# RKWin93/E2E-MAPPO-for-MT-FJSP

Hardware: AMD Instinct MI355X
Metric: env-steps/sec (batched J6M6E2) (higher is better)
Workload: dtype f64 (environment) / f32 (encoder: f32 storage and accumulation; 128x128 products on the 16-bit matrix cores from split f32 operands, f32-accurate: DESIGN.md §4)

## Files before the change

### __graft_entry__.py

```python
#!/usr/bin/env python3
import os
import sys

ROOT = os.path.dirname(os.path.abspath(__file__))
if ROOT not in sys.path:
    sys.path.insert(0, ROOT)


def build() -> None:
    from importlib import import_module
    import mtfjsp_amd
    _build = import_module("e2e-mappo-for-mt-fjsp_amd._build")
    lib = _build.build(force=True, verbose=True)
    capi = import_module("e2e-mappo-for-mt-fjsp_amd.capi")
    capi.lib()
    print("variant:", _build.build_variant("funcs", ["-DMTFJSP_BODY_FUNCS=3"]))
    from oracle import env_oracle
    print("oracle:", env_oracle.build(force=True))
    print("built", lib)


def smoke() -> None:
    import numpy as np
    import torch
    from importlib import import_module
    import mtfjsp_amd
    assert torch.cuda.is_available(), "smoke() needs cuda:0"
    batch_env = import_module("e2e-mappo-for-mt-fjsp_amd.batch_env")
    inst = import_module("e2e-mappo-for-mt-fjsp_amd.instances")
    from oracle.env_oracle import OracleBatch
    J, M, E, B = 6, 6, 2, 8
    T = J * M
    t, p, tt, edge = inst.generate_instances(B, J, M, E, seed=0)
    import random
    random.seed(0)
    w3 = inst.random_weights(B)
    env = batch_env.DeviceBatchEnv(J, M, E, B, obs_dtype="f64")
    env.load_instances(t, p, tt, edge=edge)
    env.scaler_init()
    env.reset(w3)
    orc = OracleBatch(t, p, tt, edge)
    orc.scaler_init()
    orc.reset(w3)
    a = torch.zeros(B, dtype=torch.int32, device=env.device); m = torch.zeros_like(a); j = torch.zeros_like(a)
    for s in range(T):
        env.random_actions(7, s, a, m, j)
        env.step(a, m)
        info, raw, _ = orc.step(a.cpu().numpy(), m.cpu().numpy())
        cand, mask = orc.job_mask_update(j.cpu().numpy())
# ... 25 lines not shown
```

### e2e-mappo-for-mt-fjsp_amd/csrc/mtfjsp_gin_resident.h

```cpp
#ifndef GR_KERNEL
#ifndef MTFJSP_GIN_RESIDENT_H
#define MTFJSP_GIN_RESIDENT_H
#include <type_traits>
#include <utility>
#include "mtfjsp_gin_res_select.h"

#ifndef GR_ABL
#define GR_ABL 0
#endif
#ifndef GR_NRES
#define GR_NRES 16
#endif
#ifndef GR_VRES
#define GR_VRES 1
#endif
#define GR_RING 6
#define GR_NBAR 6
#ifndef GR_GRP
#define GR_GRP 2
#endif
#ifndef GR_LOOK
#define GR_LOOK 2
#endif
#define GR_ROWB 272
#define GR_PLANE (32 * GR_ROWB)
#define GR_TILE (2 * GR_PLANE)
#define GR_MAXWARM 10
#ifndef GR_FX_DROP
#define GR_FX_DROP 1
#endif
#ifndef GR_FX_TAIL
#define GR_FX_TAIL 1
#endif
#ifndef GR_FX_SETUP
#define GR_FX_SETUP 1
#endif
struct GrShapeAny { static constexpr bool FIXED = false; static constexpr int T = 0, J = 0, IPC = 0; };
template <int T_, int J_, int IPC_> struct GrShapeFixed {
    static constexpr bool FIXED = true; static constexpr int T = T_, J = J_, IPC = IPC_;
    static_assert(T_ >= GR_MINT && T_ <= GR_MAXT && IPC_ * T_ == GR_ROWS && IPC_ * J_ <= GR_MAXCAND && (IPC_ * 128) % 256 == 0, "fixed shape: full 576-row workgroups");
};
typedef GrShapeFixed<GIN_RES_FX_T, GIN_RES_FX_J, GIN_RES_FX_IPC> GrShapeHeadline;
constexpr int gr_left_at(int T, int h, int rt)
{
    int left = ((16 * h) / T + 1) * T - 16 * h;
    for (int i = 0; i < rt; i++) { left -= 32; if (left <= 0) left += T; if (left <= 0) left += T; }
    return left;
}
constexpr int gr_max_chunks(int T)
{
    int m = 0;
    for (int i = 0; i < 16; i++) { const int r0 = i * T, c = ((r0 + T - 1) >> 4) - (r0 >> 4) + 1; m = c > m ? c : m; }
    return m;
}

#ifndef GR_MIX
#define GR_MIX 2
#endif
#ifndef GR_SETTLE
#define GR_SETTLE 1
#endif
#ifndef GR_FOLD_DPP
#define GR_FOLD_DPP 1
#endif
#ifndef GR_STAT_ASM
#define GR_STAT_ASM 0
#endif
#ifndef GR_PK
#define GR_PK 1
#endif
typedef float f32x16 __attribute__((ext_vector_type(16)));
typedef _Float16 gr_h8 __attribute__((ext_vector_type(8)));
typedef _Float16 gr_h2 __attribute__((ext_vector_type(2)));

struct GinResArgs {
    int B, T, J, ipc;
    const void *tfea; int feat_f64;
    const int *ell_col; const float *ell_val;
    const void *Wx32[6];
    float wsinv[6];
    const float *gamma[6], *beta[6];
    unsigned long long *stats;
    unsigned long long *stats_next;
    int wexp[6];
    int ffrac[6];
    unsigned long long *bar;
    unsigned long long epoch;
    unsigned *fail;
    unsigned *range_flag;
    const int *candidate;
    float *pooled;
    float *cand_feat;
    float *h_nodes;
// ... 218 lines not shown
            if (r < GR_ROWS) {
                unsigned cp = 0xffffffffu; float v0 = 0.f, v1 = 0.f;
                if (r < nrows) {
                    const int2 cc = ecc[k];
                    const float2 vv = evv[k];
                    const int base = (r / T) * T;
                    const unsigned r0 = cc.x >= 0 ? (unsigned)(base + cc.x) : 0xffffu, r1 = cc.y >= 0 ? (unsigned)(base + cc.y) : 0xffffu;
                    cp = r0 | (r1 << 16); v0 = cc.x >= 0 ? vv.x : 0.f; v1 = cc.y >= 0 ? vv.y : 0.f;
                }
                s_ellc[r] = cp; s_ellv0[r] = v0; s_ellv1[r] = v1; s_rowcand[r] = -1;
            }
        }
        {
            const f32x4 *wi = reinterpret_cast<const f32x4 *>(A.Wx32[0]) + (size_t)wave * (3 * 64) + lane;
            __builtin_amdgcn_sched_barrier(0);
#pragma unroll
            for (int p = 0; p < 3; p++) w0pre[p] = wi[p * 64];
            __builtin_amdgcn_sched_barrier(0);
        }
        if (tid == 0) s_flag[1] = 0u;
        if (tid < 5 * (GR_NT / GR_GRP)) s_cnt[tid] = 0u;
        for (int i = tid; i < 2 * GR_TILE / 16; i += 256) reinterpret_cast<float4 *>(s_planes)[i] = make_float4(0.f, 0.f, 0.f, 0.f);
        if (have_cand) {
            LDS_BARRIER();
#pragma unroll
            for (int k = 0; k < (GR_MAXCAND + 255) / 256; k++) {
                const int i = tid + 256 * k, c = cand_pre[k];
                if (i < ninst * Jn && c >= 0 && c < T && atomicExch(&s_rowcand[(i / Jn) * T + c], i) != -1) s_flag[1] = 1u;
            }
        }
        if constexpr (!FXD) s_zero[tid] = 0.f;
    }
    f32x16 acc[GR_NRES];
    f32x16 zs[2];
    float *zsp = A.zspill + ((size_t)(blockIdx.x * 4 + wave) * (GR_NT - GR_NRES)) * 1024 + lane * 4;
    auto zload = [&](auto Jc) __attribute__((always_inline)) {
        constexpr int j = decltype(Jc)::value;
        if constexpr (GR_VRES) return;
#pragma unroll
        for (int g = 0; g < 4; g++) {
            const float4 v = *reinterpret_cast<const float4 *>(zsp + j * 1024 + g * 256);
            zs[j & 1][4 * g] = v.x; zs[j & 1][4 * g + 1] = v.y; zs[j & 1][4 * g + 2] = v.z; zs[j & 1][4 * g + 3] = v.w;
        }
    };
    auto zstore = [&](auto Jc, const f32x16 &a) __attribute__((always_inline)) {
        constexpr int j = decltype(Jc)::value;
        if constexpr (GR_VRES) return;
#pragma unroll
        for (int g = 0; g < 4; g++) *reinterpret_cast<float4 *>(zsp + j * 1024 + g * 256) = make_float4(a[4 * g], a[4 * g + 1], a[4 * g + 2], a[4 * g + 3]);
    };
#define GR_TILEVAL(rt) ((rt) < GR_NRES ? acc[(rt) < GR_NRES ? (rt) : 0] : zs[(rt) >= GR_NRES ? ((rt) - GR_NRES) & 1 : 0])
    auto mfma_v = [&](f32x16 &c, const gr_h8 &a, const gr_h8 &b, bool zero) __attribute__((always_inline)) {
        if (zero) asm volatile("v_mfma_f32_32x32x16_f16 %0, %1, %2, 0" : "=v"(c) : "v"(a), "v"(b));
        else asm volatile("v_mfma_f32_32x32x16_f16 %0, %1, %2, %0" : "+v"(c) : "v"(a), "v"(b));
    };
    int nrows_l = nrows, n_l = n;
    auto bn_of = [&](int rt) __attribute__((always_inline)) -> const float * {
        if constexpr (FXD) return s_bn;
        else return rt * 32 + n_l < nrows_l ? s_bn : s_zero;
    };
    bool timed_out = false;
    gr_h8 wf[2][8];
    bf16x8 w0f[3];
    f32x2 ts[8], tq[8];
#pragma unroll
    for (int i = 0; i < 8; i++) { ts[i] = f32x2{0.f, 0.f}; tq[i] = f32x2{0.f, 0.f}; }

    auto load_weights = [&](int layer) __attribute__((always_inline)) {
        const float4 *wi = reinterpret_cast<const float4 *>(A.Wx32[layer]) + (size_t)wave * (2 * 8 * 64) + lane;
#pragma unroll
        for (int p = 0; p < 2; p++)
#pragma unroll
            for (int ks = 0; ks < 8; ks++) wf[p][ks] = __builtin_bit_cast(gr_h8, wi[(p * 8 + ks) * 64]);
    };
    auto stat2 = [&](int i, float x, float y) __attribute__((always_inline)) {
        const f32x2 v = {x, y};
#if GR_STAT_ASM == 1
        asm volatile("v_pk_add_f32 %0, %2, %0\n\tv_pk_fma_f32 %1, %2, %2, %1" : "+v"(ts[i]), "+v"(tq[i]) : "v"(v));
#elif GR_STAT_ASM == 2
        float s0 = ts[i][0], s1 = ts[i][1], q0 = tq[i][0], q1 = tq[i][1];
        asm volatile("v_add_f32 %0, %4, %0\n\tv_add_f32 %1, %5, %1\n\tv_fma_f32 %2, %4, %4, %2\n\tv_fma_f32 %3, %5, %5, %3" : "+v"(s0), "+v"(s1), "+v"(q0), "+v"(q1) : "v"(x), "v"(y));
        ts[i] = f32x2{s0, s1}; tq[i] = f32x2{q0, q1};
#else
        ts[i] = gr_add2(ts[i], v); tq[i] = gr_fma2(v, v, tq[i]);
        asm volatile("" : "+v"(ts[i]), "+v"(tq[i]));
#endif
    };
    auto stats_all = [&](const f32x16 &a) __attribute__((always_inline)) {
        if (GR_ABL & 4) return;
#pragma unroll
        for (int i = 0; i < 8; i++) stat2(i, a[2 * i], a[2 * i + 1]);
    };
    auto split2x4 = [&](f32x2 v01, f32x2 v23, uint2 &p0, uint2 &p1) __attribute__((always_inline)) {
        const gr_h2 a = __builtin_convertvector(v01, gr_h2), b = __builtin_convertvector(v23, gr_h2);
#if GR_MIX == 2
        const gr_h2 c = gr_rem16(v01, a), d = gr_rem16(v23, b);
#else
        const f32x2 r01 = gr_rem2(v01, a), r23 = gr_rem2(v23, b);
        const gr_h2 c = __builtin_convertvector(r01, gr_h2), d = __builtin_convertvector(r23, gr_h2);
#endif
        p0 = make_uint2(__builtin_bit_cast(unsigned, a), __builtin_bit_cast(unsigned, b));
        p1 = make_uint2(__builtin_bit_cast(unsigned, c), __builtin_bit_cast(unsigned, d));
    };
    auto stats_tile = [&](auto Tc) __attribute__((always_inline)) {
        constexpr int RT = decltype(Tc)::value;
        stats_all(GR_TILEVAL(RT));
// ... 18 lines not shown
    };
    auto fold_stats_dpp = [&]() __attribute__((always_inline)) {
        const bool b4 = (lane & 16) != 0, b3 = (lane & 8) != 0, b2 = (lane & 4) != 0, b1 = (lane & 2) != 0, b0 = (lane & 1) != 0;
        auto dpp = [&](float x, auto Ctrl) __attribute__((always_inline)) {
            return __builtin_bit_cast(float, __builtin_amdgcn_update_dpp(0, __builtin_bit_cast(int, x), decltype(Ctrl)::value, 0xF, 0xF, true));
        };
        float v16[16];
#pragma unroll
        for (int c = 0; c < 16; c++) {
            const float a = ts[c >> 1][c & 1], q_ = tq[c >> 1][c & 1];
            v16[c] = (b4 ? q_ : a) + __shfl_xor(b4 ? a : q_, 16);
        }
#pragma unroll
        for (int i = 0; i < 8; i++) { ts[i] = f32x2{0.f, 0.f}; tq[i] = f32x2{0.f, 0.f}; }
        float v8[8];
#pragma unroll
        for (int c = 0; c < 8; c++) v8[c] = (b3 ? v16[c + 8] : v16[c]) + dpp(b3 ? v16[c] : v16[c + 8], std::integral_constant<int, 0x140>{});
        float v4[4];
#pragma unroll
        for (int c = 0; c < 4; c++) v4[c] = (b2 ? v8[c + 4] : v8[c]) + dpp(b2 ? v8[c] : v8[c + 4], std::integral_constant<int, 0x141>{});
        float v2[2];
#pragma unroll
        for (int c = 0; c < 2; c++) v2[c] = (b1 ? v4[c + 2] : v4[c]) + dpp(b1 ? v4[c] : v4[c + 2], std::integral_constant<int, 0x4E>{});
        return (b0 ? v2[1] : v2[0]) + dpp(b0 ? v2[0] : v2[1], std::integral_constant<int, 0xB1>{});
    };
    unsigned char *const pl0 = s_planes, *const pl1 = s_planes + GR_TILE, *const plr = reinterpret_cast<unsigned char *>(s_ring);
    auto plane_buf = [&](int i) __attribute__((always_inline)) { return i == 0 ? pl0 : i == 1 ? pl1 : plr + (i - 2) * GR_TILE; };
    auto produce_quarter = [&](auto Tc, auto Gc, unsigned char *pbuf) __attribute__((always_inline)) {
        constexpr int rt = decltype(Tc)::value, g = decltype(Gc)::value;
        unsigned char *dst = pbuf + n * GR_ROWB + (32 * wave + 8 * g + 4 * h) * 2;
        const float *bn = bn_of(rt);
        const float4 s4 = *reinterpret_cast<const float4 *>(bn + 32 * wave + 8 * g + 4 * h);
        const float4 h4 = *reinterpret_cast<const float4 *>(bn + HD + 32 * wave + 8 * g + 4 * h);
        const f32x16 &a = GR_TILEVAL(rt);
        uint2 p0, p1;
        split2x4(f32x2{bn_relu_ss(a[4 * g], s4.x, h4.x), bn_relu_ss(a[4 * g + 1], s4.y, h4.y)},
                 f32x2{bn_relu_ss(a[4 * g + 2], s4.z, h4.z), bn_relu_ss(a[4 * g + 3], s4.w, h4.w)}, p0, p1);
        *reinterpret_cast<uint2 *>(dst) = p0;
        *reinterpret_cast<uint2 *>(dst + GR_PLANE) = p1;
    };
    auto produce_tile = [&](auto Tc, unsigned char *pbuf) __attribute__((always_inline)) {
        gr_static_for<4>([&](auto Gc) __attribute__((always_inline)) { produce_quarter(Tc, Gc, pbuf); });
        __builtin_amdgcn_sched_barrier(0);
    };
    const unsigned char *xa0 = s_planes + n * GR_ROWB + 16 * h;
#define GR_FENCE() __builtin_amdgcn_sched_barrier(0)
#define GR_PIN_V() do { } while (0)
    auto consume_tile = [&](auto Tc) __attribute__((always_inline)) {
        constexpr int RT = decltype(Tc)::value;
        constexpr int PT = RT + GR_LOOK;
        constexpr bool NEXT = (PT < GR_NT) && !(GR_ABL & 1);
        constexpr bool STATS = RT > 0 && (GR_VRES || RT - 1 < GR_NRES) && !(GR_ABL & 4);
        const unsigned char *xa = plane_buf(RT % (2 * GR_LOOK)) + n * GR_ROWB + 16 * h;
        unsigned char *pnext = plane_buf(PT % (2 * GR_LOOK));
        const float *bn = bn_of(PT);
        gr_h8 xf[2][2];
#pragma unroll
        for (int p = 0; p < 2; p++) xf[0][p] = *reinterpret_cast<const gr_h8 *>(xa + p * GR_PLANE);
        float4 s4 = make_float4(0.f, 0.f, 0.f, 0.f), h4 = s4;
        if constexpr (NEXT) {
            s4 = *reinterpret_cast<const float4 *>(bn + 32 * wave + 4 * h);
            h4 = *reinterpret_cast<const float4 *>(bn + HD + 32 * wave + 4 * h);
        }
        constexpr bool VT = GR_VRES && RT >= GR_NRES;
        f32x16 atmp;
        f32x16 &a = RT < GR_NRES ? acc[RT < GR_NRES ? RT : 0] : VT ? zs[RT >= GR_NRES ? (RT - GR_NRES) & 1 : 0] : atmp;
        if constexpr (RT + GR_LOOK + 1 >= GR_NRES && RT + GR_LOOK + 1 < GR_NT) zload(std::integral_constant<int, RT + GR_LOOK + 1 - GR_NRES>{});
        gr_static_for<4>([&](auto Pc) __attribute__((always_inline)) {
            constexpr int g = decltype(Pc)::value;
            const gr_h8 *x0 = xf[0], *x1 = xf[1];
            f32x2 v01 = {0.f, 0.f}, v23 = {0.f, 0.f}, e01 = v01, e23 = v01;
            gr_h2 p01 = {0, 0}, p23 = p01, q01 = p01, q23 = p01;
            unsigned char *dst = pnext + n * GR_ROWB + (32 * wave + 8 * g + 4 * h) * 2;
            const f32x16 &nx = GR_TILEVAL(PT < GR_NT ? PT : RT);
            const f32x16 &pv = GR_TILEVAL(RT > 0 ? RT - 1 : 0);
            auto M = [&](int ks, int wp, int xp) __attribute__((always_inline)) {
                if (GR_ABL & 2) return;
                if constexpr (VT) mfma_v(a, wf[wp][ks], (ks & 1) ? x1[xp] : x0[xp], ks == 0 && wp == 0 && xp == 1);
                else if (ks == 0 && wp == 0 && xp == 1)
                    a = __builtin_amdgcn_mfma_f32_32x32x16_f16(wf[wp][ks], x0[xp], f32x16{0.f, 0.f, 0.f, 0.f, 0.f, 0.f, 0.f, 0.f, 0.f, 0.f, 0.f, 0.f, 0.f, 0.f, 0.f, 0.f}, 0, 0, 0);
                else a = __builtin_amdgcn_mfma_f32_32x32x16_f16(wf[wp][ks], (ks & 1) ? x1[xp] : x0[xp], a, 0, 0, 0);
            };
            M(2 * g, 0, 1);
            xf[1][0] = *reinterpret_cast<const gr_h8 *>(xa + 32 * (2 * g + 1));
            if constexpr (NEXT) { v01 = gr_fma2(f32x2{nx[4 * g], nx[4 * g + 1]}, f32x2{s4.x, s4.y}, f32x2{h4.x, h4.y});
                                  v23 = gr_fma2(f32x2{nx[4 * g + 2], nx[4 * g + 3]}, f32x2{s4.z, s4.w}, f32x2{h4.z, h4.w}); }
            GR_FENCE();
            M(2 * g, 1, 0);
            xf[1][1] = *reinterpret_cast<const gr_h8 *>(xa + GR_PLANE + 32 * (2 * g + 1));
            if constexpr (NEXT) { v01 = __builtin_elementwise_max(v01, f32x2{0.f, 0.f}); v23 = __builtin_elementwise_max(v23, f32x2{0.f, 0.f}); }
            GR_FENCE();
            M(2 * g, 0, 0);
            if constexpr (NEXT) { p01 = __builtin_convertvector(v01, gr_h2); p23 = __builtin_convertvector(v23, gr_h2); }
            if constexpr (NEXT && g < 3) s4 = *reinterpret_cast<const float4 *>(bn + 32 * wave + 8 * (g + 1) + 4 * h);
            GR_FENCE();
            M(2 * g + 1, 0, 1);
            if constexpr (g < 3) xf[0][0] = *reinterpret_cast<const gr_h8 *>(xa + 32 * (2 * g + 2));
            if constexpr (NEXT && !GR_MIX) { e01 = __builtin_convertvector(p01, f32x2); e23 = __builtin_convertvector(p23, f32x2); }
            if constexpr (NEXT && g < 3) h4 = *reinterpret_cast<const float4 *>(bn + HD + 32 * wave + 8 * (g + 1) + 4 * h);
            GR_FENCE();
            M(2 * g + 1, 1, 0);
            if constexpr (g < 3) xf[0][1] = *reinterpret_cast<const gr_h8 *>(xa + GR_PLANE + 32 * (2 * g + 2));
            if constexpr (NEXT) { if constexpr (GR_MIX == 2) { q01 = gr_rem16(v01, p01); q23 = gr_rem16(v23, p23); }
                                  else if constexpr (GR_MIX == 1) { v01 = gr_rem2(v01, p01); v23 = gr_rem2(v23, p23); } else { v01 = gr_sub2(v01, e01); v23 = gr_sub2(v23, e23); }
                                  if (!(GR_ABL & 8)) *reinterpret_cast<uint2 *>(dst) = make_uint2(__builtin_bit_cast(unsigned, p01), __builtin_bit_cast(unsigned, p23));
                                  if constexpr (GR_MIX != 2) { q01 = __builtin_convertvector(v01, gr_h2); q23 = __builtin_convertvector(v23, gr_h2); } }
            GR_FENCE();
            M(2 * g + 1, 0, 0);
            if constexpr (NEXT) { if (!(GR_ABL & 8)) *reinterpret_cast<uint2 *>(dst + GR_PLANE) = make_uint2(__builtin_bit_cast(unsigned, q01), __builtin_bit_cast(unsigned, q23));
                                  else asm volatile("" :: "v"(p01), "v"(p23), "v"(q01), "v"(q23)); }
            if constexpr (STATS) { stat2(2 * g, pv[4 * g], pv[4 * g + 1]); stat2(2 * g + 1, pv[4 * g + 2], pv[4 * g + 3]); }
            GR_FENCE();
        });
        if constexpr (RT >= GR_NRES && !GR_VRES) {
            stats_all(a);
            zstore(std::integral_constant<int, RT - GR_NRES>{}, a);
            GR_FENCE();
        }
        if constexpr (!VT && GR_SETTLE) { asm volatile("s_nop 1"); GR_FENCE(); }
    };
    auto consume_tile0 = [&](auto Tc) __attribute__((always_inline)) {
        constexpr int RT = decltype(Tc)::value;
        const unsigned char *xa = xa0 + 32 * (RT & 7);
        bf16x8 x[3];
#pragma unroll
        for (int p = 0; p < 3; p++) x[p] = *reinterpret_cast<const bf16x8 *>(xa + p * GR_PLANE);
        f32x16 a = {0.f, 0.f, 0.f, 0.f, 0.f, 0.f, 0.f, 0.f, 0.f, 0.f, 0.f, 0.f, 0.f, 0.f, 0.f, 0.f};
        a = __builtin_amdgcn_mfma_f32_32x32x16_bf16(w0f[0], x[2], a, 0, 0, 0);
        a = __builtin_amdgcn_mfma_f32_32x32x16_bf16(w0f[2], x[0], a, 0, 0, 0);
        a = __builtin_amdgcn_mfma_f32_32x32x16_bf16(w0f[1], x[1], a, 0, 0, 0);
        a = __builtin_amdgcn_mfma_f32_32x32x16_bf16(w0f[0], x[1], a, 0, 0, 0);
        a = __builtin_amdgcn_mfma_f32_32x32x16_bf16(w0f[1], x[0], a, 0, 0, 0);
        a = __builtin_amdgcn_mfma_f32_32x32x16_bf16(w0f[0], x[0], a, 0, 0, 0);
        if constexpr (RT < GR_NRES) acc[RT] = a;
        else if constexpr (GR_VRES) zs[(RT - GR_NRES) & 1] = a;
        else {
            stats_all(a);
            zstore(std::integral_constant<int, RT - GR_NRES>{}, a);
        }
        if constexpr (RT > 0 && (GR_VRES || RT - 1 < GR_NRES)) stats_tile(std::integral_constant<int, RT - 1>{});
        __builtin_amdgcn_sched_barrier(0);
    };
    float *s_wtab = s_ring + 1024 + 4 * (2 * 32 * 36);
    static_assert(!(GR_FX_SETUP && GR_FOLD_DPP) || (1024 + 4 * (2 * 32 * 36)) * 4 >= (2 * GR_LOOK - 2) * GR_TILE, "s_wtab lies past the plane buffers in the ring area");
    unsigned warm_word = 0;
    int slot[GR_NT];
    auto final_setup_a = [&]() __attribute__((always_inline)) {
        int tid_s = tid;
        if constexpr (FXS) asm volatile("" : "+v"(tid_s));
        for (int i = tid_s; i < 17 * 16; i += 256) s_wtab[i] = (i & 15) < (i >> 4) ? 1.0f : 0.0f;
        if (A.nwarm > 0) {
            unsigned l = (blockIdx.x >> 3) * 256u + (unsigned)tid_s;
            const unsigned char *wp = reinterpret_cast<const unsigned char *>(A.warm[0]);
            bool found = false;
            for (int w = 0; w < A.nwarm; w++) {
                const unsigned nl = A.warm_lines[w];
                if (!found && l < nl) { wp = reinterpret_cast<const unsigned char *>(A.warm[w]) + (size_t)l * 128; found = true; }
                if (!found) l -= nl;
            }
            warm_word = *reinterpret_cast<const unsigned *>(wp);
        }
    };
    auto final_setup_b = [&]() __attribute__((always_inline)) {
#ifndef GR_KEEP_MASKS
        asm volatile("" : "+v"(n_l));
#endif
#pragma unroll
        for (int rt = 0; rt < GR_NT; rt++) slot[rt] = (GR_ABL & 32) ? -1 : s_rowcand[rt * 32 + n_l];
    };
    auto layer_boundary = [&](auto Kc) __attribute__((always_inline)) {
        constexpr int k = decltype(Kc)::value;
        GR_STAMP_AT(4 + 4 * k);
        if constexpr (GR_VRES && GR_NT > GR_NRES) {
            asm volatile("s_nop 15\n\ts_nop 15" ::: "memory");
            stats_all(zs[(GR_NT - 1 - GR_NRES) & 1]);
        }
#if GR_FOLD_DPP
        (void)fold_stats;
        const float colsum = fold_stats_dpp();
        int lane_b = lane;
        if constexpr (FXS && k == 5) asm volatile("" : "+v"(lane_b));
        const int n_b = lane_b & 31, h_b = lane_b >> 5;
        const int kind = n_b >> 4, scol = 32 * wave + 8 * ((n_b & 15) >> 2) + 4 * h_b + (n_b & 3);
        constexpr int PAIR = 16;
#else
        const float colsum = fold_stats();
        const int kind = tid & 1, scol = tid >> 1;
        constexpr int PAIR = 1;
#endif
        const int sidx = 2 * scol + kind;
        if (k == 1) GR_STAMP_AT(2);
        const unsigned grp = blockIdx.x & 7u;
        {
            float x = colsum;
            if (!(__builtin_fabsf(x) * (kind ? A.wsinv[k] * A.wsinv[k] : A.wsinv[k]) < __builtin_ldexpf(1.0f, 51 - A.ffrac[k]))) {
                if (A.range_flag && !timed_out) __hip_atomic_store(A.range_flag, 1u, __ATOMIC_RELAXED, __HIP_MEMORY_SCOPE_SYSTEM);
                x = 0.f;
            }
            (void)__hip_atomic_fetch_add(A.stats + ((size_t)k * 8 + grp) * 256 + sidx, gr_fix_encode(x, kind ? 2 * A.wexp[k] : A.wexp[k], A.ffrac[k]),
                                         __ATOMIC_RELAXED, __HIP_MEMORY_SCOPE_AGENT);
        }
        if (k == 1) GR_STAMP_AT(3);
        const float ga = A.gamma[k][scol], be = A.beta[k][scol];
        if constexpr (k < 5) load_weights(k + 1);
        else if constexpr (FXS) { final_setup_a(); final_setup_b(); }
        GR_STAMP_AT(5 + 4 * k);
        const unsigned long long *w0 = A.stats + (size_t)k * 8 * 256 + sidx;
        unsigned long long vw[8], want[8], ssum = 0;
#pragma unroll
        for (int j = 0; j < 8; j++) want[j] = (unsigned long long)((nblk >> 3) + ((unsigned)j < (nblk & 7u) ? 1u : 0u));
        {
            const unsigned long long t0 = __builtin_amdgcn_s_memrealtime();
            for (;;) {
#pragma unroll
                for (int j = 0; j < 8; j++) vw[j] = __hip_atomic_load(w0 + (size_t)j * 256, __ATOMIC_RELAXED, __HIP_MEMORY_SCOPE_AGENT);
                bool done = true;
                ssum = 0;
#pragma unroll
                for (int j = 0; j < 8; j++) { done = done && (vw[j] >> 58) == want[j]; ssum += vw[j] & GR_FIX_PAYLOAD; }
                if (__builtin_amdgcn_ballot_w64(!done) == 0ull) break;
                if (__builtin_amdgcn_s_memrealtime() - t0 > 400000ull) {
                    __hip_atomic_store(A.fail, 1u, __ATOMIC_RELAXED, __HIP_MEMORY_SCOPE_SYSTEM);
                    timed_out = true;
                    break;
                }
                __builtin_amdgcn_s_sleep(2);
            }
            GR_STAMP_AT(6 + 4 * k);
            const double tot = gr_fix_decode(ssum, nblk, A.ffrac[k]);
            const double oth = __shfl_xor(tot, PAIR);
            if (!kind) {
                const double mean = tot * A.inv_rows;
                double var = oth * A.inv_rows - mean * mean;
                if (var < 0) var = 0;
                const float rstd = 1.0f / sqrtf((float)(var + BN_EPS));
                const float s = rstd * ga;
                s_bn[scol] = s * A.wsinv[k];
                s_bn[HD + scol] = be - (float)mean * s;
            }
        }
        LDS_BARRIER();
        GR_STAMP_AT(7 + 4 * k);
    };

    GR_STAMP_AT(0);
#pragma unroll
    for (int p = 0; p < 3; p++) w0f[p] = __builtin_bit_cast(bf16x8, w0pre[p]);
    LDS_BARRIER();
    GR_STAMP_AT(1);
    {
        const float *s_feat = s_ring;
        auto produce0 = [&](int rt) __attribute__((always_inline)) {
            const int r = 8 * wave + (lane >> 3), fk = lane & 7, row = rt * 32 + r;
            const int fo = fk < 6 ? 2 * fk : 0;
            const unsigned cp = s_ellc[row];
            const unsigned r0 = cp & 0xffffu, r1 = cp >> 16;
            const int deg = 1 + (r0 != 0xffffu) + (r1 != 0xffffu);
            const float inv = deg == 1 ? 1.0f : deg == 2 ? 0.5f : (1.0f / 3.0f);
            const float w0 = s_ellv0[row], w1 = s_ellv1[row];
            const int n0 = r0 != 0xffffu ? (int)r0 : row, n1 = r1 != 0xffffu ? (int)r1 : row;
            const float2 o = *reinterpret_cast<const float2 *>(s_feat + row * 12 + fo);
            const float2 x = *reinterpret_cast<const float2 *>(s_feat + n0 * 12 + fo);
            const float2 y = *reinterpret_cast<const float2 *>(s_feat + n1 * 12 + fo);
            float v[4] = {__builtin_fmaf(w1, y.x, __builtin_fmaf(w0, x.x, o.x)) * inv, __builtin_fmaf(w1, y.y, __builtin_fmaf(w0, x.y, o.y)) * inv, 0.f, 0.f};
            if (!FXD && row >= nrows) { v[0] = 0.f; v[1] = 0.f; }
            uint2 p0, p1, p2;
            split3x4(v, p0, p1, p2);
            unsigned char *d = s_planes + r * GR_ROWB + 32 * (rt & 7) + 4 * fk;
            if (fk < 6) {
                *reinterpret_cast<unsigned *>(d) = p0.x;
                *reinterpret_cast<unsigned *>(d + GR_PLANE) = p1.x;
                *reinterpret_cast<unsigned *>(d + 2 * GR_PLANE) = p2.x;
            }
// ... 25 lines not shown
            gr_static_for<GR_LOOK>([&](auto Ic) __attribute__((always_inline)) { produce_tile(Ic, plane_buf(decltype(Ic)::value)); });
            LDS_BARRIER();
            unsigned *cnt = s_cnt + (layer - 1) * (GR_NT / GR_GRP);
            gr_static_for<GR_NT>([&](auto Tc) __attribute__((always_inline)) {
                constexpr int RT = decltype(Tc)::value;
                constexpr int step = RT / GR_GRP, back = GR_LOOK / GR_GRP;
                if constexpr (GR_LOOK > GR_GRP && RT % GR_GRP == 0 && step >= back) {
                    while (__builtin_amdgcn_readfirstlane(__hip_atomic_load(&cnt[step - back], __ATOMIC_RELAXED, __HIP_MEMORY_SCOPE_WORKGROUP)) < 4u)
                        __builtin_amdgcn_s_sleep(1);
                    asm volatile("" ::: "memory");
                    __builtin_amdgcn_sched_barrier(0);
                }
                consume_tile(Tc);
                GR_PIN_V();
                if constexpr (RT % GR_GRP == GR_GRP - 1) {
                    if constexpr (GR_LOOK > GR_GRP) {
                        asm volatile("" ::: "memory");
                        if (lane == 0) __hip_atomic_fetch_add(&cnt[step], 1u, __ATOMIC_RELAXED, __HIP_MEMORY_SCOPE_WORKGROUP);
                    } else LDS_BARRIER();
                }
                __builtin_amdgcn_sched_barrier(0);
            });
            if constexpr (GR_LOOK > GR_GRP) LDS_BARRIER();
            static_assert(GR_NT % GR_GRP == 0 && GR_GRP >= 1 && (GR_LOOK == GR_GRP || GR_LOOK == 2 * GR_GRP) && GR_LOOK <= GR_NRES, "tile groups");
        } else {
            auto write_h = [&](auto Tc) __attribute__((always_inline)) {
                constexpr int rt = decltype(Tc)::value;
                float *base = s_ring + ((rt % GR_RING) * 32 + n) * HD;
                gr_static_for<4>([&](auto Gc) __attribute__((always_inline)) {
                    constexpr int g = decltype(Gc)::value;
                    const float *bn = bn_of(rt);
                    const float4 s4 = *reinterpret_cast<const float4 *>(bn + 32 * wave + 8 * g + 4 * h);
                    const float4 h4 = *reinterpret_cast<const float4 *>(bn + HD + 32 * wave + 8 * g + 4 * h);
                    const f32x16 &a = GR_TILEVAL(rt);
                    const int ch = (8 * wave + 2 * g + h) ^ (n & 7);
                    *reinterpret_cast<float4 *>(base + 4 * ch) = make_float4(bn_relu_ss(a[4 * g], s4.x, h4.x), bn_relu_ss(a[4 * g + 1], s4.y, h4.y),
                                                                             bn_relu_ss(a[4 * g + 2], s4.z, h4.z), bn_relu_ss(a[4 * g + 3], s4.w, h4.w));
                });
                __builtin_amdgcn_sched_barrier(0);
            };
            auto ring_row = [&](int R) __attribute__((always_inline)) {
                const int t = R >> 5;
                return ((t - GR_RING * ((t * 43) >> 8)) * 32 + (R & 31)) * HD;
            };
            struct AggRow { const float *po, *px, *py; float w0, w1, inv; int s0, s1, s2; };
            auto agg_row = [&](int RT) __attribute__((always_inline)) {
                AggRow r;
                const int row = RT * 32 + n_l;
                const unsigned cp = s_ellc[row];
                const unsigned r0 = cp & 0xffffu, r1 = cp >> 16;
                r.w0 = s_ellv0[row]; r.w1 = s_ellv1[row];
                const int deg = 1 + (r0 != 0xffffu) + (r1 != 0xffffu);
                r.inv = deg == 1 ? 1.0f : deg == 2 ? 0.5f : (1.0f / 3.0f);
                const int n0 = r0 != 0xffffu ? (int)r0 : row, n1 = r1 != 0xffffu ? (int)r1 : row;
                r.po = s_ring + ((RT % GR_RING) * 32 + n) * HD; r.px = s_ring + ring_row(n0); r.py = s_ring + ring_row(n1);
                r.s0 = n & 7; r.s1 = n0 & 7; r.s2 = n1 & 7;
                return r;
            };
            auto agg_quarter_standalone = [&](const AggRow &r, int g, unsigned char *dst) __attribute__((always_inline)) {
                const int chl = 8 * wave + 2 * g + h;
                const float4 o = *reinterpret_cast<const float4 *>(r.po + 4 * (chl ^ r.s0));
                const float4 x = *reinterpret_cast<const float4 *>(r.px + 4 * (chl ^ r.s1));
                const float4 y = *reinterpret_cast<const float4 *>(r.py + 4 * (chl ^ r.s2));
                const f32x2 W0 = {r.w0, r.w0}, W1 = {r.w1, r.w1}, IV = {r.inv, r.inv};
                const f32x2 v01 = gr_mul2(gr_fma2(W1, f32x2{y.x, y.y}, gr_fma2(W0, f32x2{x.x, x.y}, f32x2{o.x, o.y})), IV);
                const f32x2 v23 = gr_mul2(gr_fma2(W1, f32x2{y.z, y.w}, gr_fma2(W0, f32x2{x.z, x.w}, f32x2{o.z, o.w})), IV);
                uint2 p0, p1;
                split2x4(v01, v23, p0, p1);
                *reinterpret_cast<uint2 *>(dst + 16 * g) = p0;
                *reinterpret_cast<uint2 *>(dst + 16 * g + GR_PLANE) = p1;
            };
            auto consume_agg = [&](auto Tc) __attribute__((always_inline)) {
                constexpr int RT = decltype(Tc)::value;
                constexpr bool NEXT = RT + 1 < GR_NT && !(GR_ABL & 1);
                constexpr bool WH = RT + 4 < GR_NT && !(GR_ABL & 1);
                constexpr int WT = WH ? RT + 4 : RT;
                constexpr bool STATS = RT > 0 && (GR_VRES || RT - 1 < GR_NRES) && !(GR_ABL & 4);
                constexpr bool VT = GR_VRES && RT >= GR_NRES;
                const unsigned char *xa = xa0 + (RT & 1) * GR_TILE;
                gr_h8 xf[2][2];
#pragma unroll
                for (int p = 0; p < 2; p++) xf[0][p] = *reinterpret_cast<const gr_h8 *>(xa + p * GR_PLANE);
                AggRow r = agg_row(NEXT ? RT + 1 : RT);
                unsigned char *dst = s_planes + ((RT + 1) & 1) * GR_TILE + n * GR_ROWB + (32 * wave + 4 * h) * 2;
                const float *bnw = bn_of(WT);
                float *hbase = s_ring + ((WT % GR_RING) * 32 + n) * HD;
                float4 s4 = make_float4(0.f, 0.f, 0.f, 0.f), h4 = s4;
                if constexpr (WH) {
                    s4 = *reinterpret_cast<const float4 *>(bnw + 32 * wave + 4 * h);
                    h4 = *reinterpret_cast<const float4 *>(bnw + HD + 32 * wave + 4 * h);
                }
                f32x16 atmp;
                f32x16 &a = RT < GR_NRES ? acc[RT < GR_NRES ? RT : 0] : VT ? zs[RT >= GR_NRES ? (RT - GR_NRES) & 1 : 0] : atmp;
                if constexpr (RT + 6 >= GR_NRES && RT + 6 < GR_NT) zload(std::integral_constant<int, RT + 6 - GR_NRES>{});
                gr_static_for<4>([&](auto Pc) __attribute__((always_inline)) {
                    constexpr int g = decltype(Pc)::value;
                    const gr_h8 *x0 = xf[0], *x1 = xf[1];
                    const f32x16 &wv = GR_TILEVAL(WT);
                    const f32x16 &pv = GR_TILEVAL(RT > 0 ? RT - 1 : 0);
                    const int chl = 8 * wave + 2 * g + h;
                    float4 o = make_float4(0.f, 0.f, 0.f, 0.f), x = o, y = o;
                    f32x2 v01 = {0.f, 0.f}, v23 = v01, e01 = v01, e23 = v01, u01 = v01, u23 = v01;
                    gr_h2 p01 = {0, 0}, p23 = p01, q01 = p01, q23 = p01;
                    const f32x2 W0 = {r.w0, r.w0}, W1 = {r.w1, r.w1}, IV = {r.inv, r.inv};
                    auto M = [&](int ks, int wp, int xp) __attribute__((always_inline)) {
                        if (!(GR_ABL & 2)) {
                            if constexpr (VT) mfma_v(a, wf[wp][ks], (ks & 1) ? x1[xp] : x0[xp], g == 0 && ks == 0 && wp == 0 && xp == 1);
                            else if (g == 0 && ks == 0 && wp == 0 && xp == 1)
                                a = __builtin_amdgcn_mfma_f32_32x32x16_f16(wf[wp][ks], x0[xp], f32x16{0.f, 0.f, 0.f, 0.f, 0.f, 0.f, 0.f, 0.f, 0.f, 0.f, 0.f, 0.f, 0.f, 0.f, 0.f, 0.f}, 0, 0, 0);
                            else a = __builtin_amdgcn_mfma_f32_32x32x16_f16(wf[wp][ks], (ks & 1) ? x1[xp] : x0[xp], a, 0, 0, 0);
                        }
                    };
                    M(2 * g, 0, 1);
                    xf[1][0] = *reinterpret_cast<const gr_h8 *>(xa + 32 * (2 * g + 1));
                    if constexpr (NEXT) { o = *reinterpret_cast<const float4 *>(r.po + 4 * (chl ^ r.s0)); x = *reinterpret_cast<const float4 *>(r.px + 4 * (chl ^ r.s1));
                                          y = *reinterpret_cast<const float4 *>(r.py + 4 * (chl ^ r.s2)); }
                    if constexpr (STATS) { stat2(2 * g, pv[4 * g], pv[4 * g + 1]); stat2(2 * g + 1, pv[4 * g + 2], pv[4 * g + 3]); }
                    GR_FENCE();
                    M(2 * g, 1, 0);
                    xf[1][1] = *reinterpret_cast<const gr_h8 *>(xa + GR_PLANE + 32 * (2 * g + 1));
                    if constexpr (WH) { u01 = __builtin_elementwise_max(gr_fma2(f32x2{wv[4 * g], wv[4 * g + 1]}, f32x2{s4.x, s4.y}, f32x2{h4.x, h4.y}), f32x2{0.f, 0.f});
                                        u23 = __builtin_elementwise_max(gr_fma2(f32x2{wv[4 * g + 2], wv[4 * g + 3]}, f32x2{s4.z, s4.w}, f32x2{h4.z, h4.w}), f32x2{0.f, 0.f}); }
                    GR_FENCE();
                    M(2 * g, 0, 0);
                    if constexpr (WH) *reinterpret_cast<float4 *>(hbase + 4 * (chl ^ (n & 7))) = make_float4(u01[0], u01[1], u23[0], u23[1]);
                    if constexpr (NEXT) { v01 = gr_fma2(W0, f32x2{x.x, x.y}, f32x2{o.x, o.y}); v23 = gr_fma2(W0, f32x2{x.z, x.w}, f32x2{o.z, o.w}); }
                    if constexpr (WH && g < 3) s4 = *reinterpret_cast<const float4 *>(bnw + 32 * wave + 8 * (g + 1) + 4 * h);
                    GR_FENCE();
                    M(2 * g + 1, 0, 1);
                    if constexpr (g < 3) xf[0][0] = *reinterpret_cast<const gr_h8 *>(xa + 32 * (2 * g + 2));
                    if constexpr (NEXT) { v01 = gr_fma2(W1, f32x2{y.x, y.y}, v01); v23 = gr_fma2(W1, f32x2{y.z, y.w}, v23); }
                    if constexpr (WH && g < 3) h4 = *reinterpret_cast<const float4 *>(bnw + HD + 32 * wave + 8 * (g + 1) + 4 * h);
                    GR_FENCE();
                    M(2 * g + 1, 1, 0);
                    if constexpr (g < 3) xf[0][1] = *reinterpret_cast<const gr_h8 *>(xa + GR_PLANE + 32 * (2 * g + 2));
                    if constexpr (NEXT) { v01 = gr_mul2(v01, IV); v23 = gr_mul2(v23, IV); p01 = __builtin_convertvector(v01, gr_h2); p23 = __builtin_convertvector(v23, gr_h2);
                                          if constexpr (!GR_MIX) { e01 = __builtin_convertvector(p01, f32x2); e23 = __builtin_convertvector(p23, f32x2); } }
                    GR_FENCE();
                    M(2 * g + 1, 0, 0);
                    if constexpr (NEXT) { if constexpr (GR_MIX == 2) { q01 = gr_rem16(v01, p01); q23 = gr_rem16(v23, p23); }
                                          else { if constexpr (GR_MIX) { v01 = gr_rem2(v01, p01); v23 = gr_rem2(v23, p23); } else { v01 = gr_sub2(v01, e01); v23 = gr_sub2(v23, e23); } q01 = __builtin_convertvector(v01, gr_h2); q23 = __builtin_convertvector(v23, gr_h2); }
                                          *reinterpret_cast<uint2 *>(dst + 16 * g) = make_uint2(__builtin_bit_cast(unsigned, p01), __builtin_bit_cast(unsigned, p23));
                                          *reinterpret_cast<uint2 *>(dst + 16 * g + GR_PLANE) = make_uint2(__builtin_bit_cast(unsigned, q01), __builtin_bit_cast(unsigned, q23)); }
                    GR_FENCE();
                });
                if constexpr (RT >= GR_NRES && !GR_VRES) {
                    stats_all(a);
                    zstore(std::integral_constant<int, RT - GR_NRES>{}, a);
                    GR_FENCE();
                }
                if constexpr (!VT && GR_SETTLE) { asm volatile("s_nop 1"); GR_FENCE(); }
            };
            write_h(std::integral_constant<int, 0>{}); write_h(std::integral_constant<int, 1>{}); write_h(std::integral_constant<int, 2>{});
            write_h(std::integral_constant<int, 3>{});
            LDS_BARRIER();
            {
                const AggRow r = agg_row(0);
                unsigned char *dst = s_planes + n * GR_ROWB + (32 * wave + 4 * h) * 2;
#pragma unroll
                for (int g = 0; g < 4; g++) agg_quarter_standalone(r, g, dst);
            }
            LDS_BARRIER();
            __builtin_amdgcn_sched_barrier(0);
            gr_static_for<GR_NT>([&](auto Tc) __attribute__((always_inline)) {
                consume_agg(Tc);
                LDS_BARRIER();
                __builtin_amdgcn_sched_barrier(0);
            });
        }
        layer_boundary(std::integral_constant<int, layer>{});
    });

    GR_STAMP_AT(30);
    {
        int lane_f = lane;
        asm volatile("" : "+v"(lane_f));
        const int n_f = lane_f & 31, h_f = lane_f >> 5;
        float *s_part = reinterpret_cast<float *>(s_planes);
        static_assert(2 * GR_NT * 2 * HD * 4 <= 2 * GR_TILE + 4096, "partial pool sums: plane buffers + 4 KB");
        float *tb = s_ring + 1024 + wave * (2 * 32 * 36);
        if constexpr (!FXS) final_setup_a();
        float4 S[4], Hs[4];
#pragma unroll
        for (int g = 0; g < 4; g++) {
// ... 20 lines not shown
            constexpr int rt = decltype(Rc)::value;
            const int lf = left_at(Rc);
            const float *rb = tb + (rt & 1) * (32 * 36) + (16 * h_f) * 36 + c;
#pragma unroll
            for (int i = 0; i < 16; i++) x[i] = rb[i * 36];
            const float4 *wt = reinterpret_cast<const float4 *>(s_wtab + (lf < 16 ? lf : 16) * 16);
            w0 = wt[0]; w1 = wt[1]; w2 = wt[2]; w3 = wt[3];
        };
        auto pool_math = [&](auto Rc) __attribute__((always_inline)) {
            constexpr int rt = decltype(Rc)::value;
            const int lf = left_at(Rc);
            f32x2 sa2 = gr_fma2(f32x2{x[0], x[1]}, f32x2{w0.x, w0.y}, f32x2{0.f, 0.f});
            sa2 = gr_fma2(f32x2{x[2], x[3]}, f32x2{w0.z, w0.w}, sa2);
            sa2 = gr_fma2(f32x2{x[4], x[5]}, f32x2{w1.x, w1.y}, sa2);
            sa2 = gr_fma2(f32x2{x[6], x[7]}, f32x2{w1.z, w1.w}, sa2);
            sa2 = gr_fma2(f32x2{x[8], x[9]}, f32x2{w2.x, w2.y}, sa2);
            sa2 = gr_fma2(f32x2{x[10], x[11]}, f32x2{w2.z, w2.w}, sa2);
            sa2 = gr_fma2(f32x2{x[12], x[13]}, f32x2{w3.x, w3.y}, sa2);
            sa2 = gr_fma2(f32x2{x[14], x[15]}, f32x2{w3.z, w3.w}, sa2);
            const f32x2 t2 = gr_add2(gr_add2(gr_add2(f32x2{x[0], x[1]}, f32x2{x[2], x[3]}), gr_add2(f32x2{x[4], x[5]}, f32x2{x[6], x[7]})),
                                     gr_add2(gr_add2(f32x2{x[8], x[9]}, f32x2{x[10], x[11]}), gr_add2(f32x2{x[12], x[13]}, f32x2{x[14], x[15]})));
            const float tot = t2[0] + t2[1];
            const float sa = sa2[0] + sa2[1];
            float *pp = s_part + ((2 * rt + h_f) * 2) * HD + 32 * wave + c;
            pp[0] = lf >= 16 ? tot : sa; pp[HD] = lf >= 16 ? 0.f : tot - sa;
            if constexpr (!FXD) {
                left -= 32;
                if (left <= 0) left += T;
                if (left <= 0) left += T;
            }
        };
        gr_static_for<GR_NT>([&](auto Tc) __attribute__((always_inline)) {
            constexpr int rt = decltype(Tc)::value;
            const f32x16 &a = GR_TILEVAL(rt);
            if constexpr (rt > 0) { if (!(GR_ABL & 16)) pool_load(std::integral_constant<int, rt - 1>{}); }
            float4 v[4];
#pragma unroll
            for (int g = 0; g < 4; g++) {
                const f32x2 lo = __builtin_elementwise_max(gr_fma2(f32x2{a[4 * g], a[4 * g + 1]}, f32x2{S[g].x, S[g].y}, f32x2{Hs[g].x, Hs[g].y}), f32x2{0.f, 0.f});
                const f32x2 hi = __builtin_elementwise_max(gr_fma2(f32x2{a[4 * g + 2], a[4 * g + 3]}, f32x2{S[g].z, S[g].w}, f32x2{Hs[g].z, Hs[g].w}), f32x2{0.f, 0.f});
                v[g] = make_float4(lo[0], lo[1], hi[0], hi[1]);
            }
            float *wb = tb + (rt & 1) * (32 * 36);
#pragma unroll
            for (int g = 0; g < 4; g++) *reinterpret_cast<float4 *>(wb + n_f * 36 + 8 * g + 4 * h_f) = v[g];
            if (slot[rt] >= 0) {
                float *d = FXD ? reinterpret_cast<float *>(cbase + ((unsigned)slot[rt] * (unsigned)(HD * 4) + coff))
                               : A.cand_feat + ((size_t)inst0 * Jn + slot[rt]) * HD + 32 * wave + 4 * h_f;
#pragma unroll
                for (int g = 0; g < 4; g++) *reinterpret_cast<float4 *>(d + 8 * g) = v[g];
            }
            if (!FXD && A.h_nodes && rt * 32 + n_l < nrows) {
                float *d = A.h_nodes + (grow0 + rt * 32 + n_l) * HD + 32 * wave + 4 * h_f;
#pragma unroll
                for (int g = 0; g < 4; g++) *reinterpret_cast<float4 *>(d + 8 * g) = v[g];
            }
            if constexpr (rt > 0) { if (!(GR_ABL & 16)) pool_math(std::integral_constant<int, rt - 1>{}); }
            __builtin_amdgcn_sched_barrier(0);
        });
        if (!(GR_ABL & 16)) { pool_load(std::integral_constant<int, GR_NT - 1>{}); pool_math(std::integral_constant<int, GR_NT - 1>{}); }
        asm volatile("" :: "v"(warm_word));
        GR_STAMP_AT(29);
        LDS_BARRIER();
        const float invT = 1.0f / (float)T;
        static_assert(GR_MAXT <= 65, "an instance spans at most five 16-row chunks");
        if constexpr (FXT) {
// ... 56 lines not shown
```

Baseline: 21.57 million.

## Place resident accumulators and weight fragments in AGPRs via inline-asm MFMA

Adds a GR_AW mode, on by default, that keeps the first ten resident accumulator tiles and the f16 weight fragments in accumulation registers (AGPRs). It does this with inline-asm MFMA and global loads whose constraints target AGPRs, plus explicit waits for the weight loads before the barrier. The remaining tiles live in VGPR spill slots, since NRES drops from 16 to 10. The aim is to free arch VGPRs and cut register pressure or spills in the persistent GIN encoder kernel. In exchange it adds AGPR-to-VGPR moves at every elementwise touch of a tile and longer s_nop settle padding. It also keeps more tiles on the VGPR path.

```diff
diff --git a/__graft_entry__.py b/__graft_entry__.py
--- a/__graft_entry__.py
+++ b/__graft_entry__.py
@@ -15,6 +15,7 @@
     capi = import_module("e2e-mappo-for-mt-fjsp_amd.capi")
     capi.lib()
     print("variant:", _build.build_variant("funcs", ["-DMTFJSP_BODY_FUNCS=3"]))
+    print("variant:", _build.build_variant("aw0", ["-DGR_AW=0", "-DGR_NRES=16"]))
     from oracle import env_oracle
     print("oracle:", env_oracle.build(force=True))
     print("built", lib)
diff --git a/e2e-mappo-for-mt-fjsp_amd/csrc/mtfjsp_gin_resident.h b/e2e-mappo-for-mt-fjsp_amd/csrc/mtfjsp_gin_resident.h
--- a/e2e-mappo-for-mt-fjsp_amd/csrc/mtfjsp_gin_resident.h
+++ b/e2e-mappo-for-mt-fjsp_amd/csrc/mtfjsp_gin_resident.h
@@ -8,8 +8,11 @@
 #ifndef GR_ABL
 #define GR_ABL 0
 #endif
+#ifndef GR_AW
+#define GR_AW 1
+#endif
 #ifndef GR_NRES
-#define GR_NRES 16
+#define GR_NRES (GR_AW ? 10 : 16)
 #endif
 #ifndef GR_VRES
 #define GR_VRES 1
@@ -59,6 +62,9 @@
 #endif
 #ifndef GR_SETTLE
 #define GR_SETTLE 1
+#endif
+#ifndef GR_AW_SETTLE_T
+#define GR_AW_SETTLE_T 0
 #endif
 #ifndef GR_FOLD_DPP
 #define GR_FOLD_DPP 1
@@ -343,7 +349,9 @@
         if constexpr (!FXD) s_zero[tid] = 0.f;
     }
     f32x16 acc[GR_NRES];
-    f32x16 zs[2];
+    static_assert(GR_VRES || GR_NT - GR_NRES == 2, "the round trip through zspill stages exactly two tiles");
+#define GR_ZIDX(rt) ((rt) < GR_NRES ? 0 : GR_VRES ? (rt) - GR_NRES : ((rt) - GR_NRES) & 1)
+    f32x16 zs[GR_VRES ? (GR_NT - GR_NRES > 0 ? GR_NT - GR_NRES : 1) : 2];
     float *zsp = A.zspill + ((size_t)(blockIdx.x * 4 + wave) * (GR_NT - GR_NRES)) * 1024 + lane * 4;
     auto zload = [&](auto Jc) __attribute__((always_inline)) {
         constexpr int j = decltype(Jc)::value;
@@ -360,16 +368,29 @@
 #pragma unroll
         for (int g = 0; g < 4; g++) *reinterpret_cast<float4 *>(zsp + j * 1024 + g * 256) = make_float4(a[4 * g], a[4 * g + 1], a[4 * g + 2], a[4 * g + 3]);
     };
-#define GR_TILEVAL(rt) ((rt) < GR_NRES ? acc[(rt) < GR_NRES ? (rt) : 0] : zs[(rt) >= GR_NRES ? ((rt) - GR_NRES) & 1 : 0])
+#define GR_TILEVAL(rt) ((rt) < GR_NRES ? acc[(rt) < GR_NRES ? (rt) : 0] : zs[GR_ZIDX(rt)])
+#if GR_AW
+    auto mfma_v = [&](f32x16 &c, const gr_h8 &a, const gr_h8 &b, bool zero) __attribute__((always_inline)) {
+        if (zero) asm volatile("v_mfma_f32_32x32x16_f16 %0, %1, %2, 0" : "=&v"(c) : "a"(a), "v"(b));
+        else asm volatile("v_mfma_f32_32x32x16_f16 %0, %1, %2, %0" : "+v"(c) : "a"(a), "v"(b));
+    };
+    auto mfma_a = [&](f32x16 &c, const gr_h8 &a, const gr_h8 &b, bool zero) __attribute__((always_inline)) {
+        if (zero) asm volatile("v_mfma_f32_32x32x16_f16 %0, %1, %2, 0" : "=&a"(c) : "a"(a), "v"(b));
+        else asm volatile("v_mfma_f32_32x32x16_f16 %0, %1, %2, %0" : "+a"(c) : "a"(a), "v"(b));
+    };
+#else
     auto mfma_v = [&](f32x16 &c, const gr_h8 &a, const gr_h8 &b, bool zero) __attribute__((always_inline)) {
         if (zero) asm volatile("v_mfma_f32_32x32x16_f16 %0, %1, %2, 0" : "=v"(c) : "v"(a), "v"(b));
         else asm volatile("v_mfma_f32_32x32x16_f16 %0, %1, %2, %0" : "+v"(c) : "v"(a), "v"(b));
     };
+#endif
     int nrows_l = nrows, n_l = n;
     auto bn_of = [&](int rt) __attribute__((always_inline)) -> const float * {
         if constexpr (FXD) return s_bn;
         else return rt * 32 + n_l < nrows_l ? s_bn : s_zero;
     };
+    auto tile_touch = [&](f32x16 &c) __attribute__((always_inline)) { asm volatile("" : "+a"(c)); };
+#define GR_TOUCH(rt) do { if constexpr (GR_AW && (rt) < GR_NRES) tile_touch(acc[(rt) < GR_NRES ? (rt) : 0]); } while (0)
     bool timed_out = false;
     gr_h8 wf[2][8];
     bf16x8 w0f[3];
@@ -379,10 +400,26 @@
 
     auto load_weights = [&](int layer) __attribute__((always_inline)) {
         const float4 *wi = reinterpret_cast<const float4 *>(A.Wx32[layer]) + (size_t)wave * (2 * 8 * 64) + lane;
+#if GR_AW
+#pragma unroll
+        for (int q = 0; q < 4; q++) {
+            const float4 *wq = wi + q * (4 * 64);
+            asm volatile("global_load_dwordx4 %0, %4, off\n\tglobal_load_dwordx4 %1, %4, off offset:1024\n\t"
+                         "global_load_dwordx4 %2, %4, off offset:2048\n\tglobal_load_dwordx4 %3, %4, off offset:3072"
+                         : "=&a"(wf[q >> 1][4 * (q & 1)]), "=&a"(wf[q >> 1][4 * (q & 1) + 1]), "=&a"(wf[q >> 1][4 * (q & 1) + 2]), "=&a"(wf[q >> 1][4 * (q & 1) + 3])
+                         : "v"(wq) : "memory");
+        }
+#else
 #pragma unroll
         for (int p = 0; p < 2; p++)
 #pragma unroll
             for (int ks = 0; ks < 8; ks++) wf[p][ks] = __builtin_bit_cast(gr_h8, wi[(p * 8 + ks) * 64]);
+#endif
+    };
+    auto weights_arrived = [&]() __attribute__((always_inline)) {
+#if GR_AW
+        asm volatile("s_waitcnt vmcnt(0)" ::: "memory");
+#endif
     };
     auto stat2 = [&](int i, float x, float y) __attribute__((always_inline)) {
         const f32x2 v = {x, y};
@@ -467,6 +504,7 @@
         const float *bn = bn_of(rt);
         const float4 s4 = *reinterpret_cast<const float4 *>(bn + 32 * wave + 8 * g + 4 * h);
         const float4 h4 = *reinterpret_cast<const float4 *>(bn + HD + 32 * wave + 8 * g + 4 * h);
+        GR_TOUCH(rt);
         const f32x16 &a = GR_TILEVAL(rt);
         uint2 p0, p1;
         split2x4(f32x2{bn_relu_ss(a[4 * g], s4.x, h4.x), bn_relu_ss(a[4 * g + 1], s4.y, h4.y)},
@@ -499,7 +537,7 @@
         }
         constexpr bool VT = GR_VRES && RT >= GR_NRES;
         f32x16 atmp;
-        f32x16 &a = RT < GR_NRES ? acc[RT < GR_NRES ? RT : 0] : VT ? zs[RT >= GR_NRES ? (RT - GR_NRES) & 1 : 0] : atmp;
+        f32x16 &a = RT < GR_NRES ? acc[RT < GR_NRES ? RT : 0] : VT ? zs[GR_ZIDX(RT)] : atmp;
         if constexpr (RT + GR_LOOK + 1 >= GR_NRES && RT + GR_LOOK + 1 < GR_NT) zload(std::integral_constant<int, RT + GR_LOOK + 1 - GR_NRES>{});
         gr_static_for<4>([&](auto Pc) __attribute__((always_inline)) {
             constexpr int g = decltype(Pc)::value;
@@ -512,13 +550,18 @@
             auto M = [&](int ks, int wp, int xp) __attribute__((always_inline)) {
                 if (GR_ABL & 2) return;
                 if constexpr (VT) mfma_v(a, wf[wp][ks], (ks & 1) ? x1[xp] : x0[xp], ks == 0 && wp == 0 && xp == 1);
+#if GR_AW
+                else mfma_a(a, wf[wp][ks], (ks & 1) ? x1[xp] : x0[xp], ks == 0 && wp == 0 && xp == 1);
+#else
                 else if (ks == 0 && wp == 0 && xp == 1)
                     a = __builtin_amdgcn_mfma_f32_32x32x16_f16(wf[wp][ks], x0[xp], f32x16{0.f, 0.f, 0.f, 0.f, 0.f, 0.f, 0.f, 0.f, 0.f, 0.f, 0.f, 0.f, 0.f, 0.f, 0.f, 0.f}, 0, 0, 0);
                 else a = __builtin_amdgcn_mfma_f32_32x32x16_f16(wf[wp][ks], (ks & 1) ? x1[xp] : x0[xp], a, 0, 0, 0);
+#endif
             };
             M(2 * g, 0, 1);
             xf[1][0] = *reinterpret_cast<const gr_h8 *>(xa + 32 * (2 * g + 1));
-            if constexpr (NEXT) { v01 = gr_fma2(f32x2{nx[4 * g], nx[4 * g + 1]}, f32x2{s4.x, s4.y}, f32x2{h4.x, h4.y});
+            if constexpr (NEXT) { GR_TOUCH(PT < GR_NT ? PT : RT);
+                                  v01 = gr_fma2(f32x2{nx[4 * g], nx[4 * g + 1]}, f32x2{s4.x, s4.y}, f32x2{h4.x, h4.y});
                                   v23 = gr_fma2(f32x2{nx[4 * g + 2], nx[4 * g + 3]}, f32x2{s4.z, s4.w}, f32x2{h4.z, h4.w}); }
             GR_FENCE();
             M(2 * g, 1, 0);
@@ -544,7 +587,7 @@
             M(2 * g + 1, 0, 0);
             if constexpr (NEXT) { if (!(GR_ABL & 8)) *reinterpret_cast<uint2 *>(dst + GR_PLANE) = make_uint2(__builtin_bit_cast(unsigned, q01), __builtin_bit_cast(unsigned, q23));
                                   else asm volatile("" :: "v"(p01), "v"(p23), "v"(q01), "v"(q23)); }
-            if constexpr (STATS) { stat2(2 * g, pv[4 * g], pv[4 * g + 1]); stat2(2 * g + 1, pv[4 * g + 2], pv[4 * g + 3]); }
+            if constexpr (STATS) { GR_TOUCH(RT > 0 ? RT - 1 : 0); stat2(2 * g, pv[4 * g], pv[4 * g + 1]); stat2(2 * g + 1, pv[4 * g + 2], pv[4 * g + 3]); }
             GR_FENCE();
         });
         if constexpr (RT >= GR_NRES && !GR_VRES) {
@@ -552,7 +595,8 @@
             zstore(std::integral_constant<int, RT - GR_NRES>{}, a);
             GR_FENCE();
         }
-        if constexpr (!VT && GR_SETTLE) { asm volatile("s_nop 1"); GR_FENCE(); }
+        if constexpr (!VT && GR_SETTLE && !GR_AW) { asm volatile("s_nop 1"); GR_FENCE(); }
+        if constexpr (GR_AW && GR_AW_SETTLE_T) { asm volatile("s_nop 15"); GR_FENCE(); }
     };
     auto consume_tile0 = [&](auto Tc) __attribute__((always_inline)) {
         constexpr int RT = decltype(Tc)::value;
@@ -568,7 +612,7 @@
         a = __builtin_amdgcn_mfma_f32_32x32x16_bf16(w0f[1], x[0], a, 0, 0, 0);
         a = __builtin_amdgcn_mfma_f32_32x32x16_bf16(w0f[0], x[0], a, 0, 0, 0);
         if constexpr (RT < GR_NRES) acc[RT] = a;
-        else if constexpr (GR_VRES) zs[(RT - GR_NRES) & 1] = a;
+        else if constexpr (GR_VRES) zs[GR_ZIDX(RT)] = a;
         else {
             stats_all(a);
             zstore(std::integral_constant<int, RT - GR_NRES>{}, a);
@@ -608,13 +652,13 @@
         GR_STAMP_AT(4 + 4 * k);
         if constexpr (GR_VRES && GR_NT > GR_NRES) {
             asm volatile("s_nop 15\n\ts_nop 15" ::: "memory");
-            stats_all(zs[(GR_NT - 1 - GR_NRES) & 1]);
+            stats_all(zs[GR_ZIDX(GR_NT - 1)]);
         }
 #if GR_FOLD_DPP
         (void)fold_stats;
         const float colsum = fold_stats_dpp();
         int lane_b = lane;
-        if constexpr (FXS && k == 5) asm volatile("" : "+v"(lane_b));
+        if constexpr (GR_AW || (FXS && k == 5)) asm volatile("" : "+v"(lane_b));
         const int n_b = lane_b & 31, h_b = lane_b >> 5;
         const int kind = n_b >> 4, scol = 32 * wave + 8 * ((n_b & 15) >> 2) + 4 * h_b + (n_b & 3);
         constexpr int PAIR = 16;
@@ -674,6 +718,7 @@
                 s_bn[HD + scol] = be - (float)mean * s;
             }
         }
+        if constexpr (k < 5) weights_arrived();
         LDS_BARRIER();
         GR_STAMP_AT(7 + 4 * k);
     };
@@ -765,6 +810,7 @@
                     const float *bn = bn_of(rt);
                     const float4 s4 = *reinterpret_cast<const float4 *>(bn + 32 * wave + 8 * g + 4 * h);
                     const float4 h4 = *reinterpret_cast<const float4 *>(bn + HD + 32 * wave + 8 * g + 4 * h);
+                    GR_TOUCH(rt);
                     const f32x16 &a = GR_TILEVAL(rt);
                     const int ch = (8 * wave + 2 * g + h) ^ (n & 7);
                     *reinterpret_cast<float4 *>(base + 4 * ch) = make_float4(bn_relu_ss(a[4 * g], s4.x, h4.x), bn_relu_ss(a[4 * g + 1], s4.y, h4.y),
@@ -824,7 +870,7 @@
                     h4 = *reinterpret_cast<const float4 *>(bnw + HD + 32 * wave + 4 * h);
                 }
                 f32x16 atmp;
-                f32x16 &a = RT < GR_NRES ? acc[RT < GR_NRES ? RT : 0] : VT ? zs[RT >= GR_NRES ? (RT - GR_NRES) & 1 : 0] : atmp;
+                f32x16 &a = RT < GR_NRES ? acc[RT < GR_NRES ? RT : 0] : VT ? zs[GR_ZIDX(RT)] : atmp;
                 if constexpr (RT + 6 >= GR_NRES && RT + 6 < GR_NT) zload(std::integral_constant<int, RT + 6 - GR_NRES>{});
                 gr_static_for<4>([&](auto Pc) __attribute__((always_inline)) {
                     constexpr int g = decltype(Pc)::value;
@@ -839,20 +885,25 @@
                     auto M = [&](int ks, int wp, int xp) __attribute__((always_inline)) {
                         if (!(GR_ABL & 2)) {
                             if constexpr (VT) mfma_v(a, wf[wp][ks], (ks & 1) ? x1[xp] : x0[xp], g == 0 && ks == 0 && wp == 0 && xp == 1);
+#if GR_AW
+                            else mfma_a(a, wf[wp][ks], (ks & 1) ? x1[xp] : x0[xp], g == 0 && ks == 0 && wp == 0 && xp == 1);
+#else
                             else if (g == 0 && ks == 0 && wp == 0 && xp == 1)
                                 a = __builtin_amdgcn_mfma_f32_32x32x16_f16(wf[wp][ks], x0[xp], f32x16{0.f, 0.f, 0.f, 0.f, 0.f, 0.f, 0.f, 0.f, 0.f, 0.f, 0.f, 0.f, 0.f, 0.f, 0.f, 0.f}, 0, 0, 0);
                             else a = __builtin_amdgcn_mfma_f32_32x32x16_f16(wf[wp][ks], (ks & 1) ? x1[xp] : x0[xp], a, 0, 0, 0);
+#endif
                         }
                     };
                     M(2 * g, 0, 1);
                     xf[1][0] = *reinterpret_cast<const gr_h8 *>(xa + 32 * (2 * g + 1));
                     if constexpr (NEXT) { o = *reinterpret_cast<const float4 *>(r.po + 4 * (chl ^ r.s0)); x = *reinterpret_cast<const float4 *>(r.px + 4 * (chl ^ r.s1));
                                           y = *reinterpret_cast<const float4 *>(r.py + 4 * (chl ^ r.s2)); }
-                    if constexpr (STATS) { stat2(2 * g, pv[4 * g], pv[4 * g + 1]); stat2(2 * g + 1, pv[4 * g + 2], pv[4 * g + 3]); }
+                    if constexpr (STATS) { GR_TOUCH(RT > 0 ? RT - 1 : 0); stat2(2 * g, pv[4 * g], pv[4 * g + 1]); stat2(2 * g + 1, pv[4 * g + 2], pv[4 * g + 3]); }
                     GR_FENCE();
                     M(2 * g, 1, 0);
                     xf[1][1] = *reinterpret_cast<const gr_h8 *>(xa + GR_PLANE + 32 * (2 * g + 1));
-                    if constexpr (WH) { u01 = __builtin_elementwise_max(gr_fma2(f32x2{wv[4 * g], wv[4 * g + 1]}, f32x2{s4.x, s4.y}, f32x2{h4.x, h4.y}), f32x2{0.f, 0.f});
+                    if constexpr (WH) { GR_TOUCH(WT);
+                                        u01 = __builtin_elementwise_max(gr_fma2(f32x2{wv[4 * g], wv[4 * g + 1]}, f32x2{s4.x, s4.y}, f32x2{h4.x, h4.y}), f32x2{0.f, 0.f});
                                         u23 = __builtin_elementwise_max(gr_fma2(f32x2{wv[4 * g + 2], wv[4 * g + 3]}, f32x2{s4.z, s4.w}, f32x2{h4.z, h4.w}), f32x2{0.f, 0.f}); }
                     GR_FENCE();
                     M(2 * g, 0, 0);
@@ -882,7 +933,8 @@
                     zstore(std::integral_constant<int, RT - GR_NRES>{}, a);
                     GR_FENCE();
                 }
-                if constexpr (!VT && GR_SETTLE) { asm volatile("s_nop 1"); GR_FENCE(); }
+                if constexpr (!VT && GR_SETTLE && !GR_AW) { asm volatile("s_nop 1"); GR_FENCE(); }
+                if constexpr (GR_AW) { asm volatile("s_nop 15"); GR_FENCE(); }
             };
             write_h(std::integral_constant<int, 0>{}); write_h(std::integral_constant<int, 1>{}); write_h(std::integral_constant<int, 2>{});
             write_h(std::integral_constant<int, 3>{});
@@ -969,6 +1021,7 @@
         };
         gr_static_for<GR_NT>([&](auto Tc) __attribute__((always_inline)) {
             constexpr int rt = decltype(Tc)::value;
+            GR_TOUCH(rt);
             const f32x16 &a = GR_TILEVAL(rt);
             if constexpr (rt > 0) { if (!(GR_ABL & 16)) pool_load(std::integral_constant<int, rt - 1>{}); }
             float4 v[4];
```

Result: slower. 21.10 million (-2.2%).
